# src-d/kmcuda

Hardware: NVIDIA H100
Metric: kmeans_assign_points_per_sec (higher is better)
Workload: dtype f16 tensor-core filter (f32 accumulate) + f32 exact re-check

## Files before the change

kmcuda_b200/csrc/assign_tc.cu:

```cuda
#include <cuda.h>
#include <cuda_fp16.h>

#include <cstdio>
#include <algorithm>
#include <cstring>
#include <map>
#include <mutex>
#include <tuple>
#include <vector>

#include <cub/cub.cuh>

#include "exact.cuh"
#include "kernels.h"
#include "sm90_ptx.cuh"

namespace kmb {

namespace tc {
constexpr int TM = 128;
constexpr int TN = 128;
constexpr int KB = 64;
constexpr int MAX_NKB = 8;
constexpr int WIDE_NKB = 4;
constexpr int B_STAGES = 4;
constexpr int A_KB_BYTES = TM * 128;
constexpr int B_KB_BYTES = TN * 128;
constexpr int B_STAGE_BYTES = B_KB_BYTES;
constexpr int AUG_A_BYTES = TM * 32;
constexpr int AUG_B_BYTES = TN * 32;
constexpr int LIST_LEN = 5;
#ifndef KMB_KO
#define KMB_KO 0
#endif
#ifndef KMB_PREP_FUSED
#define KMB_PREP_FUSED 1
#endif
constexpr int FIRST_EMIT_WARP = 0;
constexpr int FIRST_CONV_WARP = 4;
constexpr int FIRST_EPI_WARP = 8;
constexpr int WARP_B_PRODUCER = 16;
constexpr int N_CONV_WARPS = 4;
constexpr int N_EPI_WARPS = 8;
constexpr int N_EMIT_WARPS = 4;
constexpr int N_THREADS = 17 * 32;
constexpr int MAX_CAND = 32;
constexpr int KNN_CAP = 40;
constexpr int KNN_MAX_KK = 16;
constexpr float SENTINEL_GUARD = -65000.f;

enum { CNT_PAIRS = 0, CNT_ROWQ = 1, CNT_OVF = 2, CNT_ERR = 3, CNT_N = 4 };

struct Stats {
  float scale;
  float cmax;
  float dcmax;
  uint32_t csq_max_bits;
  uint32_t force_exact;
  float yabs;
  float mun;
  float knn_extra;
};

constexpr uint32_t LIST_ARRAY = 2 * LIST_LEN * 256 * 4;
struct SmemLayout {
  uint32_t a, b, aug_a, aug_b, list, norms, fin, mu, bars, total;
};

__host__ __device__ constexpr bool wide_nkb(int nkb) { return nkb > WIDE_NKB; }
__host__ __device__ constexpr int b_stages(int nkb) { return wide_nkb(nkb) ? 2 : B_STAGES; }
__host__ __device__ constexpr int aug_bufs(int nkb) { return nkb <= 2 ? 2 : 1; }
__host__ __device__ constexpr int a_slots(int nkb) { return nkb <= 2 ? 4 : nkb == 3 ? 5 : nkb == 4 ? 6 : MAX_NKB; }
__host__ __device__ constexpr int norm_depth(int nkb) { return a_slots(nkb) / nkb + 1; }

__host__ __device__ constexpr SmemLayout smem_layout(int nkb) {
  SmemLayout L{};
  uint32_t o = 0;
  L.a = o; o += a_slots(nkb) * A_KB_BYTES;
  L.b = o; o += b_stages(nkb) * B_STAGE_BYTES;
  L.aug_a = o; o += AUG_A_BYTES;
  L.aug_b = o; o += aug_bufs(nkb) * AUG_B_BYTES;
  L.list = o; o += 4 * LIST_ARRAY;
  L.fin = o; o += 2 * 5 * 256 * 4;
  L.norms = o; o += norm_depth(nkb) * 4 * TM * 4;
  L.mu = o; o += MAX_NKB * KB * 4;
  L.bars = o; o += 64 * 8;
  L.total = o;
  return L;
}
static_assert(4 * LIST_ARRAY + 2 * 5 * 256 * 4 >= 48 * 256 * 4, "k-NN scratch overlaps the norms");
__host__ __device__ constexpr bool layouts_fit() {
  for (int k = 1; k <= MAX_NKB; k++)
    if (smem_layout(k).total + 1024 > 232448 || a_slots(k) < k || a_slots(k) > MAX_NKB || norm_depth(k) * k <= a_slots(k))
      return false;
  return true;
}
static_assert(layouts_fit(), "227 KiB of shared memory per block on H100; a whole tile in the A ring; norms ring depth");

enum {
  BAR_B_FULL = 0,
  BAR_B_EMPTY = BAR_B_FULL + B_STAGES,
  BAR_AUG_FULL = BAR_B_EMPTY + B_STAGES,
  BAR_AUG_EMPTY = BAR_AUG_FULL + 2,
  BAR_A_FULL = BAR_AUG_EMPTY + 2,
  BAR_A_FREE = BAR_A_FULL + MAX_NKB,
  BAR_EMIT_FULL = BAR_A_FREE + MAX_NKB,
  BAR_EMIT_EMPTY = BAR_EMIT_FULL + 2,
  BAR_COUNT = BAR_EMIT_EMPTY + 2
};
static_assert(BAR_COUNT <= 63, "barrier array too small");

struct Params {
  uint32_t n;
  int D;
  uint32_t K;
  int nkb;
  int nt;
  uint32_t ntiles;
  const __half* aug_blob;
  const Stats* stats;
  uint32_t* result;
  uint32_t* pair_row;
  uint32_t* pair_cand;
  uint32_t max_pairs;
  uint32_t* rowq;
  uint32_t* ovf_rows;
  uint32_t* counters;
  int metric;
  const float* neg_mu_s;
  uint32_t* assign;
  uint32_t* prev;
  uint32_t* d_changed;
  const uint32_t* yy_qgroup;
  const uint32_t* yy_groups;
  const uint32_t* yy_assign;
  float* yy_bounds;
  uint32_t G;
  const float* X;
  const uint32_t* rows;
  const uint32_t* d_nrows;
  const uint32_t* d_ntiles;
  const uint32_t* tile_nrows;
  const uint32_t* blk_cluster;
// ... 360 lines not shown
      const float v = __ldcg(a.csq + c);
      if (v == v && v < 3.0e38f) best = max(best, __float_as_uint(fmaxf(v, 0.f)));
    }
    for (int o = 16; o > 0; o >>= 1) best = max(best, __shfl_xor_sync(0xffffffffu, best, o));
    if (lane == 0 && best) atomicMax(&a.stats->csq_max_bits, best);
    prep_grid_barrier(a.barrier, gridDim.x);
  }

  const bool have_mu = a.metric == 0 && a.centred;
  if (warp == 0) {
    float cmax = __fsqrt_ru(__uint_as_float(__ldcg(&a.stats->csq_max_bits)));
    float s = 1.f;
    if (cmax > 0.f && cmax < 3.0e38f) {
      int e;
      frexpf(cmax, &e);
      s = ldexpf(1.f, 6 - e);
    }
    if (lane == 0) s_scale = s;
    if (blockIdx.x == 0) {
      const int Dp = a.nkb * KB;
      float m2 = 0.f;
      for (int f = lane; f < Dp; f += 32) {
        const float m = (have_mu && f < D) ? s_mu[f] : 0.f;
        a.neg_mu_s[f] = -m * s;
        m2 = fmaf(m * s, m * s, m2);
      }
      for (int o = 16; o > 0; o >>= 1) m2 += __shfl_xor_sync(0xffffffffu, m2, o);
      if (lane == 0) {
        a.stats->scale = s;
        a.stats->cmax = cmax * s * 1.001f;
        a.stats->mun = __fsqrt_ru(m2) * 1.002f;
      }
    }
  }
  __syncthreads();
  const float s = s_scale;
  for (uint32_t row = gw; row < a.rows_pad; row += nw)
    prep_table_row(row, lane, s, a.metric, a.C, nsq, K, D, a.nkb, a.table, a.aug_blob, a.stats, a.gather,
                   have_mu ? s_mu : nullptr, a.by_source);
}

#define TC_WAIT(bar, parity, site) \
  ptx::mbar_wait(bars_u32 + 8u * static_cast<uint32_t>(bar), (parity), p.counters + CNT_ERR, site, bars_u32 + 8u * 63u)

__device__ __forceinline__ uint32_t commit_assignment(uint32_t* __restrict__ assign, uint32_t* __restrict__ prev,
                                                      uint64_t row, uint32_t winner) {
  const uint32_t a = assign[row];
  prev[row] = a;
  if (a == winner) return 0u;
  assign[row] = winner;
  return 1u;
}

__device__ __forceinline__ uint32_t compact_list(uint32_t* lst, uint32_t cnt, float thr) {
  constexpr uint32_t A = LIST_ARRAY / 4;
  uint32_t w = 0;
  for (uint32_t i = 0; i < cnt; i++) {
    const uint32_t cmb = lst[i * 256];
    if (__uint_as_float(cmb) >= thr) {
      if (w != i) {
        lst[w * 256] = cmb;
        lst[A + w * 256] = lst[A + i * 256];
        lst[2 * A + w * 256] = lst[2 * A + i * 256];
        lst[3 * A + w * 256] = lst[3 * A + i * 256];
      }
      w++;
    }
  }
  return w;
}

template <int MODE>
struct BlockIter {
  uint32_t cur, lo, hi, left;
  const uint2* rg;
  __device__ __forceinline__ BlockIter(const Params& p, uint32_t tile) {
    if (MODE == 2) {
      left = p.knn_nblk[tile];
      rg = p.knn_ranges + p.knn_roff[tile];
      if (left) { lo = cur = rg->x; hi = rg->y; } else { lo = cur = hi = 0; }
    } else {
      left = static_cast<uint32_t>(p.nt);
      lo = cur = 0;
      hi = left - 1;
      rg = nullptr;
    }
  }
  __device__ __forceinline__ bool valid() const { return left != 0; }
  __device__ __forceinline__ bool seg_first() const { return cur == lo; }
  __device__ __forceinline__ bool seg_last() const { return cur == hi; }
  __device__ __forceinline__ void next() {
    left--;
    if (MODE != 2) { cur++; return; }
    if (cur == hi && left) { rg++; lo = cur = rg->x; hi = rg->y; } else { cur++; }
  }
};

__device__ __noinline__ float knn_topk_insert(float* col, int kk, float v) {
  int j = kk - 1;
  while (j > 0 && col[(j - 1) * 256] < v) {
    col[j * 256] = col[(j - 1) * 256];
    j--;
  }
  col[j * 256] = v;
  return col[(kk - 1) * 256];
}
__device__ __noinline__ void knn_select_buckets(const float* mine, const float* partner, int kk, float goff,
                                                float* out) {
  unsigned long long taken = 0ull;
  for (int o = 0; o < kk; o++) {
    float best = -INFINITY;
    int bi = -1;
    for (int j = 0; j < 64; j++) {
      const float v = j < 32 ? mine[j * 256] : partner[(j - 32) * 256];
      if (!((taken >> j) & 1ull) && v > best) { best = v; bi = j; }
    }
    if (bi >= 0) taken |= 1ull << bi;
// ... 193 lines not shown
                nx2 = ptx::ffma2(b23, b23, nx2);
                const uint64_t d01 = ptx::fsub2(a01, b01), d23 = ptx::fsub2(a23, b23);
                nd2 = ptx::ffma2(d01, d01, nd2);
                nd2 = ptx::ffma2(d23, d23, nd2);
              } else {
                nx2 = ptx::ffma2(a01, a01, nx2);
                nx2 = ptx::ffma2(a23, a23, nx2);
              }
              if (MODE == 2) {
                const float q4 = fmaf(a0, a0, fmaf(a1, a1, fmaf(a2_, a2_, a3 * a3)));
                const float y = q4 - a2c, t = a2 + y;
                a2c = (t - a2) - y;
                a2 = t;
              }
              pk[half * 16 + c * 2] = *reinterpret_cast<uint32_t*>(&h0);
              pk[half * 16 + c * 2 + 1] = *reinterpret_cast<uint32_t*>(&h1);
            }
          }
          TC_WAIT(BAR_A_FREE + as, aph ^ 1, 7);
#if KMB_KO != 3
          uint8_t* a_row = smem + L.a + as * A_KB_BYTES + row * 128;
#pragma unroll
          for (int c = 0; c < 8; c++)
            *reinterpret_cast<uint4*>(a_row + ((c ^ (row & 7)) << 4)) =
                make_uint4(pk[4 * c], pk[4 * c + 1], pk[4 * c + 2], pk[4 * c + 3]);
#else
          (void)pk;
#endif
          if (kb == nkb - 1) {
            float* norms = reinterpret_cast<float*>(smem + L.norms) + (si % NDEPTH) * 4 * TM;
            float nxl, nxh, ndl, ndh;
            ptx::unpack2(nx2, nxl, nxh);
            ptx::unpack2(nd2, ndl, ndh);
            norms[row] = nxl + nxh;
            if (MEASURED_RESIDUAL) norms[TM + row] = ndl + ndh;
            if (MODE == 2) {
              norms[2 * TM + row] = a2;
              norms[3 * TM + row] = nraw * s * s;
            }
          }
          ptx::fence_proxy_async_smem();
          __syncwarp();
          if (lane == 0) ptx::mbar_arrive(&bars[BAR_A_FULL + as]);
          if (++as == ASLOTS) { as = 0; aph ^= 1; }
        }
      }
    }
  } else if (warp >= FIRST_EPI_WARP && warp < FIRST_EPI_WARP + N_EPI_WARPS) {
    const int e = warp - FIRST_EPI_WARP;
    const int g = e >> 2, wq = e & 3;
    const int h = (lane & 3) >> 1;
    const int row = g * 64 + wq * 16 + (lane >> 2) + 8 * (lane & 1);
    const int slot = h * TM + row;
    const uint64_t adesc0 = ptx::make_smem_desc(ptx::smem_u32(smem + L.a + g * (64 * 128)), 16, 1024, 1);
    const uint64_t bdesc0 = ptx::make_smem_desc(ptx::smem_u32(smem + L.b), 16, 1024, 1);
    const uint64_t aug_ad = ptx::make_smem_desc(ptx::smem_u32(smem + L.aug_a + g * 1024), TM * 16, 128, 0);
    const uint64_t aug_bd0 = ptx::make_smem_desc(ptx::smem_u32(smem + L.aug_b), TN * 16, 128, 0);
    uint32_t bs = 0, bph = 0;
    uint32_t a_ready_si = 0xFFFFFFFFu;
    uint32_t a0 = 0, aph0 = 0;
    const float cmax = p.stats->cmax, dcmax = p.stats->dcmax;
    const float mun = MODE == 2 ? 0.f : p.stats->mun;
    const float knn_extra = MODE == 2 ? p.stats->knn_extra : 0.f;
    const float cap = p.metric == 1 ? p.stats->scale * p.stats->scale : INFINITY;
    uint32_t ac = 0, ti = 0, si = 0;
    for (uint32_t tile = tile_begin; tile < tile_end; tile += gridDim.x) {
      if (MODE == 2 && p.knn_nblk[tile] == 0) continue;
      const int par = ti & 1;
      uint32_t* lst = reinterpret_cast<uint32_t*>(smem + L.list) + par * LIST_LEN * 256 + slot;
      float* fin = reinterpret_cast<float*>(smem + L.fin) + par * 5 * 256;
      if (MODE < 2) TC_WAIT(BAR_EMIT_EMPTY + par, ((ti >> 1) & 1) ^ 1, 11);
      float M = -INFINITY, M2 = -INFINITY, margin = 0.f;
      uint32_t cnt = 0, flags = 0;
      float* topk = reinterpret_cast<float*>(smem + L.list) + slot;
      uint32_t kslot = 0;
      bool klive = false;
      uint4* kent = nullptr;
      float goff = 0.f, mmax = 0.f;
      float xa2lo = 0.f;
      uint32_t gown = UINT32_MAX;
      uint32_t* yb = nullptr;
      bool ylive = false;
      if (MODE == 3) {
        const uint64_t grow = static_cast<uint64_t>(tile) * TM + row;
        ylive = grow < p.n;
        if (ylive) {
          const uint32_t a = p.yy_assign[grow];
          if (a < p.K) gown = p.yy_groups[a];
          yb = reinterpret_cast<uint32_t*>(p.yy_bounds + grow * (p.G + 1) + 1);
        }
      }
      uint32_t seg = 0;
      if (MODE == 2) {
        klive = static_cast<uint32_t>(row) < p.tile_nrows[tile];
        kslot = (tile * TM + row) * 2u + h;
        kent = p.knn_entries + static_cast<size_t>(kslot) * KNN_CAP;
        if (p.knn_first_pass || !klive) {
          for (int j = 0; j < p.kk; j++) topk[j * 256] = -INFINITY;
          if (p.knn_first_pass)
            for (int j = 0; j < 32; j++) topk[(16 + j) * 256] = -INFINITY;
        } else {
          for (int j = 0; j < p.kk; j++) topk[j * 256] = p.knn_topk[static_cast<size_t>(j) * p.knn_stride + kslot];
          cnt = p.knn_cnt[kslot];
          flags = p.knn_flags[kslot];
        }
        M = topk[(p.kk - 1) * 256];
      }
      for (BlockIter<MODE> it(p, tile); it.valid(); it.next(), ac++) {
        const int n = static_cast<int>(it.cur);
        const int buf = ac % AUGB;
        const uint32_t aph = (ac / AUGB) & 1;
        const bool need_a = a_ready_si != si;
        const bool free_a = it.seg_last();
        a_ready_si = si;
        __syncwarp();
        float acc[64];
        uint32_t sa_prev = 0;
#pragma unroll
        for (int kb = 0; kb < NKB; kb++) {
          const bool wrap = a0 + kb >= static_cast<uint32_t>(ASLOTS);
          const uint32_t sa = wrap ? a0 + kb - ASLOTS : a0 + kb;
          if (need_a) TC_WAIT(BAR_A_FULL + sa, wrap ? aph0 ^ 1 : aph0, 4);
          TC_WAIT(BAR_B_FULL + bs, bph, 5);
          __syncwarp();
#if KMB_KO != 2
          ptx::wgmma_fence_acc(acc);
          ptx::wgmma_fence();
          const uint64_t ad = adesc0 + ((sa * A_KB_BYTES) >> 4);
          const uint64_t bd = bdesc0 + ((bs * B_STAGE_BYTES) >> 4);
#pragma unroll
          for (int k = 0; k < 4; k++) ptx::wgmma_m64n128k16(acc, ad + 2 * k, bd + 2 * k, (kb | k) ? 1u : 0u);
          ptx::wgmma_commit();
          ptx::wgmma_fence_acc(acc);
#endif
          if (kb > 0) {
            ptx::wgmma_wait<1>();
            if (lane == 0) {
              ptx::mbar_arrive(&bars[BAR_B_EMPTY + (bs ? bs - 1 : BST - 1)]);
              if (free_a) ptx::mbar_arrive(&bars[BAR_A_FREE + sa_prev]);
            }
          }
          sa_prev = sa;
          if (++bs == BST) { bs = 0; bph ^= 1; }
        }
        TC_WAIT(BAR_AUG_FULL + buf, aph, 6);
        __syncwarp();
#if KMB_KO != 2
        ptx::wgmma_fence_acc(acc);
        ptx::wgmma_fence();
        ptx::wgmma_m64n128k16(acc, aug_ad, aug_bd0 + buf * (AUG_B_BYTES >> 4), 1u);
        ptx::wgmma_commit();
#endif
        ptx::wgmma_wait<0>();
#if KMB_KO != 2
        ptx::wgmma_fence_acc(acc);
#endif
        if (lane == 0) {
          ptx::mbar_arrive(&bars[BAR_B_EMPTY + (bs ? bs - 1 : BST - 1)]);
          ptx::mbar_arrive(&bars[BAR_AUG_EMPTY + buf]);
          if (free_a) ptx::mbar_arrive(&bars[BAR_A_FREE + sa_prev]);
        }
        if (free_a) {
          a0 += NKB;
          if (a0 >= static_cast<uint32_t>(ASLOTS)) { a0 -= ASLOTS; aph0 ^= 1; }
        }
        uint32_t r0[32], r1[32];
#if KMB_KO != 1
        regroup_quad(acc, lane, r0, r1);
#else
        for (int jj = 0; jj < 32; jj++) {
          r0[jj] = __float_as_uint(-64.f * static_cast<float>(n * 128 + h * 64 + jj + 1));
          r1[jj] = __float_as_uint(-64.f * static_cast<float>(n * 128 + h * 64 + 32 + jj + 1));
        }
#endif
        if (it.seg_first()) {
          const float* norms = reinterpret_cast<const float*>(smem + L.norms) + (si % NDEPTH) * 4 * TM;
          float nx, nd;
          if (MEASURED_RESIDUAL) {
            nx = __fsqrt_ru(norms[row]) * 1.0001f;
            nd = __fsqrt_ru(norms[TM + row]) * 1.0001f;
          } else {
            const float na = __fsqrt_ru(norms[row]) * 1.0001f;
            nd = na * 4.8834e-4f + __fsqrt_ru(static_cast<float>(p.nkb * KB)) * 2.99e-8f;
            nx = na + nd;
            if (!(na < 65000.f)) flags |= 1u;
          }
          const float xn = nx + nd;
          float E = nx * dcmax + nd * cmax + nd * dcmax;
          E += static_cast<float>(p.nkb * KB + 16) * 2.4e-7f * nx * cmax;
          const float xu = xn + mun, cu = cmax + mun;
          if (MODE == 0) {
            E += 6.0e-7f * (cu * cu + xu * cu);
          } else if (MODE == 2) {
            E += 2.0e-6f * (cu * cu + xu * cu) + 2.0e-6f * xu * xu;
          } else {
            E += 2.0e-6f * (xn + cmax) * (xn + cmax) + 2.4e-7f * (xn * cmax + cmax * cmax);
          }
          if (MODE == 3) {
            xa2lo = norms[row] * (1.f - 1.0e-4f);
            if (!(nx * cmax < 6.0e4f)) flags |= 1u;
          }
          if (MODE == 2) {
            goff = 0.5f * norms[2 * TM + row];
            E += 1.2e-7f * (__fsqrt_ru(norms[3 * TM + row]) * cmax + p.stats->yabs * xn) + 4.8e-7f * (goff + xn * cmax);
          }
          margin = 2.f * E * 1.001f + 1e-30f;
          if (MODE == 2) margin += knn_extra;
          if (!(margin < 1.0e30f)) flags |= 1u;
          if (MODE == 2) {
            mmax = fmaxf(mmax, margin);
            if (p.knn_first_pass && seg == 1) {
              float mg[KNN_MAX_KK];
              __syncwarp();
              knn_select_buckets(topk + 16 * 256, reinterpret_cast<float*>(smem + L.list) + ((1 - h) * TM + row) + 16 * 256,
                                 p.kk, goff, mg);
              __syncwarp();
              for (int j = 0; j < p.kk; j++) topk[j * 256] = mg[j];
              M = mg[p.kk - 1];
            }
          }
        }
#ifdef KMB_DEBUG_SCORES
        if (MODE == 0 && p.dbg_scores) {
          const uint64_t grow = static_cast<uint64_t>(tile) * TM + row;
          float* dst = p.dbg_scores + grow * (static_cast<uint64_t>(nt) * TN) + n * TN + h * 64;
          for (int jj = 0; jj < 32; jj++) dst[jj] = __uint_as_float(r0[jj]);
          for (int jj = 0; jj < 32; jj++) dst[32 + jj] = __uint_as_float(r1[jj]);
        }
#endif
        if (MODE == 3) {
          float qm[16];
#pragma unroll
          for (int i = 0; i < 8; i++) {
            qm[i] = fmaxf(ptx::fmax3(__uint_as_float(r0[4 * i]), __uint_as_float(r0[4 * i + 1]), __uint_as_float(r0[4 * i + 2])),
                          __uint_as_float(r0[4 * i + 3]));
            qm[8 + i] = fmaxf(ptx::fmax3(__uint_as_float(r1[4 * i]), __uint_as_float(r1[4 * i + 1]), __uint_as_float(r1[4 * i + 2])),
                              __uint_as_float(r1[4 * i + 3]));
          }
          uint32_t gq[16];
          {
            const uint4* src = reinterpret_cast<const uint4*>(p.yy_qgroup) + (static_cast<size_t>(n) * 2 + h) * 4;
#pragma unroll
            for (int i = 0; i < 4; i++) {
              const uint4 v = __ldg(src + i);
              gq[4 * i] = v.x; gq[4 * i + 1] = v.y; gq[4 * i + 2] = v.z; gq[4 * i + 3] = v.w;
            }
          }
          const float Eb = 0.5f * margin;
          const float sc = p.stats->scale;
          const float inv_s = 1.f / sc, inv_s2 = inv_s * inv_s;
          const bool emit_ok = ylive && !(flags & 1u);
          float run = qm[0];
#pragma unroll
          for (int i = 1; i <= 16; i++) {
            if (i == 16 || gq[i] != gq[i - 1]) {
              const uint32_t g = gq[i - 1];
              if (emit_ok && g < p.G && g != gown) {
                float v;
                if (p.metric == 1) {
                  const float dot = fminf(1.f, fmaxf(-1.f, (run + Eb) * inv_s2));
                  v = fmaxf(0.f, acosf(dot) - 4.0e-6f);
                } else {
                  const float t = xa2lo - 2.f * (run + Eb);
                  v = t > 0.f ? __fsqrt_rd(t) * inv_s * (1.f - 4.0e-6f) : 0.f;
                }
                atomicMin(yb + g, __float_as_uint(v));
              }
              if (i < 16) run = qm[i];
            } else {
              run = fmaxf(run, qm[i]);
            }
          }
          if (it.seg_last()) si++;
          continue;
        }
        float t0[8], t1[8];
        float cm0, cm1;
#if KMB_KO == 7
        if (MODE == 0) {
          uint32_t x0 = 0, x1 = 0;
#pragma unroll
          for (int jj = 0; jj < 32; jj += 8) { x0 ^= r0[jj]; x1 ^= r1[jj]; }
          M = fmaxf(M, __uint_as_float(x0 & x1 & 0x3fffffffu));
          if (it.seg_last()) si++;
          continue;
        }
#endif
        if (MODE == 2) {
#pragma unroll
          for (int i = 0; i < 8; i++) {
            t0[i] = fmaxf(fmaxf(__uint_as_float(r0[4 * i]), __uint_as_float(r0[4 * i + 1])),
                          fmaxf(__uint_as_float(r0[4 * i + 2]), __uint_as_float(r0[4 * i + 3])));
            t1[i] = fmaxf(fmaxf(__uint_as_float(r1[4 * i]), __uint_as_float(r1[4 * i + 1])),
                          fmaxf(__uint_as_float(r1[4 * i + 2]), __uint_as_float(r1[4 * i + 3])));
          }
          cm0 = fmaxf(fmaxf(fmaxf(t0[0], t0[1]), fmaxf(t0[2], t0[3])), fmaxf(fmaxf(t0[4], t0[5]), fmaxf(t0[6], t0[7])));
          cm1 = fmaxf(fmaxf(fmaxf(t1[0], t1[1]), fmaxf(t1[2], t1[3])), fmaxf(fmaxf(t1[4], t1[5]), fmaxf(t1[6], t1[7])));
        } else {
          float u0[10], u1[10];
#pragma unroll
          for (int i = 0; i < 10; i++) {
            u0[i] = ptx::fmax3(__uint_as_float(r0[3 * i]), __uint_as_float(r0[3 * i + 1]), __uint_as_float(r0[3 * i + 2]));
            u1[i] = ptx::fmax3(__uint_as_float(r1[3 * i]), __uint_as_float(r1[3 * i + 1]), __uint_as_float(r1[3 * i + 2]));
          }
          const float w00 = ptx::fmax3(u0[0], u0[1], u0[2]), w01 = ptx::fmax3(u0[3], u0[4], u0[5]);
          const float w02 = ptx::fmax3(u0[6], u0[7], u0[8]), w03 = ptx::fmax3(u0[9], __uint_as_float(r0[30]), __uint_as_float(r0[31]));
          const float w10 = ptx::fmax3(u1[0], u1[1], u1[2]), w11 = ptx::fmax3(u1[3], u1[4], u1[5]);
          const float w12 = ptx::fmax3(u1[6], u1[7], u1[8]), w13 = ptx::fmax3(u1[9], __uint_as_float(r1[30]), __uint_as_float(r1[31]));
          cm0 = fmaxf(ptx::fmax3(w00, w01, w02), w03);
          cm1 = fmaxf(ptx::fmax3(w10, w11, w12), w13);
        }
        float thr;
        if (MODE == 0) {
          M = fmaxf(M, fmaxf(cm0, cm1));
          thr = fminf(M, cap) - margin;
        } else if (MODE == 1) {
          M2 = fmaxf(M2, fminf(M, cm0));
          M = fmaxf(M, cm0);
          M2 = fmaxf(M2, fminf(M, cm1));
          M = fmaxf(M, cm1);
          thr = fminf(M2, cap) - margin;
        } else {
          if (p.knn_first_pass && seg == 0) {
            float* bk = topk + (16 + 16 * (n & 1)) * 256;
#pragma unroll
            for (int i = 0; i < 8; i++) {
              bk[i * 256] = fmaxf(bk[i * 256], t0[i]);
              bk[(8 + i) * 256] = fmaxf(bk[(8 + i) * 256], t1[i]);
            }
          } else if (!p.knn_first_pass) {
            const float lim = M + goff;
            if (cm0 > lim) {
#pragma unroll
              for (int i = 0; i < 8; i++)
                if (t0[i] - goff > M) M = knn_topk_insert(topk, p.kk, t0[i] - goff);
            }
            if (cm1 > lim) {
#pragma unroll
              for (int i = 0; i < 8; i++)
                if (t1[i] - goff > M) M = knn_topk_insert(topk, p.kk, t1[i] - goff);
            }
          }
          thr = (M - margin) + goff;
        }
        uint32_t nc0, nc1;
        {
          const uint64_t nthr2 = ptx::pack2(-thr, -thr);
          uint32_t c00 = 0, c01 = 0, c10 = 0, c11 = 0;
#pragma unroll
          for (int jj = 0; jj < 32; jj += 2) {
            float x0, y0, x1, y1;
            ptx::unpack2(ptx::fadd2(ptx::pack2(__uint_as_float(r0[jj]), __uint_as_float(r0[jj + 1])), nthr2), x0, y0);
            ptx::unpack2(ptx::fadd2(ptx::pack2(__uint_as_float(r1[jj]), __uint_as_float(r1[jj + 1])), nthr2), x1, y1);
            if (jj < 16) {
              c00 = __funnelshift_l(__float_as_uint(x0), c00, 1);
              c00 = __funnelshift_l(__float_as_uint(y0), c00, 1);
              c10 = __funnelshift_l(__float_as_uint(x1), c10, 1);
              c10 = __funnelshift_l(__float_as_uint(y1), c10, 1);
            } else {
              c01 = __funnelshift_l(__float_as_uint(x0), c01, 1);
              c01 = __funnelshift_l(__float_as_uint(y0), c01, 1);
              c11 = __funnelshift_l(__float_as_uint(x1), c11, 1);
              c11 = __funnelshift_l(__float_as_uint(y1), c11, 1);
            }
          }
          nc0 = (c00 << 16) | c01;
          nc1 = (c10 << 16) | c11;
        }
        const uint32_t mask0 = __brev(~nc0), mask1 = __brev(~nc1);
        if (MODE == 2) {
          if (klive && !(p.knn_first_pass && seg == 0)) {
            if (mask0)
              cnt = knn_append(kent, cnt, M, cm0 - goff, mask0, static_cast<uint32_t>(n) * 4 + h * 2, margin, &flags);
            if (mask1)
              cnt = knn_append(kent, cnt, M, cm1 - goff, mask1, static_cast<uint32_t>(n) * 4 + h * 2 + 1, margin, &flags);
          }
          if (it.seg_last()) { si++; seg++; }
          continue;
        }
        if (it.seg_last()) si++;
        if (mask0 | mask1) {
          constexpr uint32_t A = LIST_ARRAY / 4;
          if (cnt >= LIST_LEN - 1) cnt = compact_list(lst, cnt, thr);
          if (cnt < LIST_LEN) {
            lst[cnt * 256] = __float_as_uint(fmaxf(cm0, cm1));
            lst[A + cnt * 256] = mask0;
            lst[2 * A + cnt * 256] = mask1;
            lst[3 * A + cnt * 256] = static_cast<uint32_t>(n);
            cnt++;
          } else {
            flags |= 2u;
          }
        }
      }
      if (MODE == 2) {
        if (klive) {
          for (int j = 0; j < p.kk; j++) p.knn_topk[static_cast<size_t>(j) * p.knn_stride + kslot] = topk[j * 256];
          p.knn_cnt[kslot] = cnt;
          p.knn_flags[kslot] = flags;
          const float sc = p.stats->scale;
          const float d2 = fmaxf(0.f, -2.f * (M - mmax));
          p.knn_dub[kslot] = (M > -INFINITY && !flags) ? __fsqrt_ru(d2) / sc * 1.0001f : INFINITY;
        }
        ti++;
        continue;
      }
      if (MODE == 3) {
        if (ylive && (flags & 1u) && h == 0)
          p.ovf_rows[atomicAdd(&p.counters[CNT_OVF], 1u)] = static_cast<uint32_t>(tile * TM + row);
        ti++;
        continue;
      }
      fin[slot] = M;
      reinterpret_cast<uint32_t*>(fin)[256 + slot] = cnt;
      reinterpret_cast<uint32_t*>(fin)[512 + slot] = flags;
      fin[768 + slot] = margin;
      if (MODE == 1) fin[1024 + slot] = M2;
      __syncwarp();
      if (lane == 0) ptx::mbar_arrive(&bars[BAR_EMIT_FULL + par]);
      ti++;
    }
  } else if (warp >= FIRST_EMIT_WARP && warp < FIRST_EMIT_WARP + N_EMIT_WARPS && MODE < 2) {
    const int row = (warp - FIRST_EMIT_WARP) * 32 + lane;
    const float cap = p.metric == 1 ? p.stats->scale * p.stats->scale : INFINITY;
    const uint32_t force = p.stats->force_exact ? 16u : 0u;
    uint32_t ti = 0, nchanged = 0;
    for (uint32_t tile = tile_begin; tile < tile_end; tile += gridDim.x, ti++) {
      const int par = ti & 1;
      const uint32_t* lst = reinterpret_cast<const uint32_t*>(smem + L.list) + par * LIST_LEN * 256;
      const float* fin = reinterpret_cast<const float*>(smem + L.fin) + par * 5 * 256;
      const uint32_t* finu = reinterpret_cast<const uint32_t*>(fin);
      TC_WAIT(BAR_EMIT_FULL + par, (ti >> 1) & 1, 12);
      uint64_t grow = static_cast<uint64_t>(tile) * TM + row;
      uint32_t cand[MAX_CAND];
      uint32_t total = 0, fl = 0;
      const bool live = grow < n_eff;
      if (MODE == 1 && live) grow = p.rows[grow];
      if (live) {
        float Mf = fmaxf(fin[row], fin[TM + row]);
        if (MODE == 1)
          Mf = fmaxf(fminf(fin[row], fin[TM + row]), fmaxf(fin[1024 + row], fin[1024 + TM + row]));
        const float thr = fminf(Mf, cap) - fin[768 + row];
        fl = finu[512 + row] | finu[512 + TM + row] | force;
        if (p.metric == 1 && !(Mf >= fin[768 + row] - cap)) fl |= 8u;
        if (!(thr > SENTINEL_GUARD)) fl |= 8u;
        for (int hh = 0; hh < 2; hh++) {
          const int sl = hh * TM + row;
          const uint32_t c2 = finu[256 + sl];
          for (uint32_t i = 0; i < c2; i++) {
            constexpr uint32_t A = LIST_ARRAY / 4;
            if (!(__uint_as_float(lst[i * 256 + sl]) >= thr)) continue;
            const uint32_t base = lst[3 * A + i * 256 + sl] * TN + hh * 64;
#pragma unroll
            for (int c = 0; c < 2; c++) {
              uint32_t m = lst[(1 + c) * A + i * 256 + sl];
              while (m) {
                const int b = __ffs(m) - 1;
                m &= m - 1;
                const uint32_t col = base + c * 32 + b;
                if (col < p.K) {
                  if (total < MAX_CAND) cand[total] = col;
                  total++;
                }
              }
            }
          }
        }
      }
      __syncwarp();
      if (lane == 0) ptx::mbar_arrive(&bars[BAR_EMIT_EMPTY + par]);
      const bool overflow = live && (fl || total > MAX_CAND || (MODE == 1 && total == 0));
      const bool multi = live && !overflow && total >= (MODE == 1 ? 1u : 2u);
      uint32_t want = multi ? total : 0, pre = want;
#pragma unroll
      for (int o = 1; o < 32; o <<= 1) {
        uint32_t v = __shfl_up_sync(0xffffffffu, pre, o);
        if (lane >= o) pre += v;
      }
      const uint32_t warp_total = __shfl_sync(0xffffffffu, pre, 31);
      const unsigned mmask = __ballot_sync(0xffffffffu, multi);
      uint32_t base = 0, rqbase = 0;
      if (lane == 0 && warp_total) {
        base = atomicAdd(&p.counters[CNT_PAIRS], warp_total);
        rqbase = atomicAdd(&p.counters[CNT_ROWQ], static_cast<uint32_t>(__popc(mmask)));
      }
      base = __shfl_sync(0xffffffffu, base, 0) + (pre - want);
      rqbase = __shfl_sync(0xffffffffu, rqbase, 0) + __popc(mmask & ((1u << lane) - 1));
      if (live) {
        if (overflow) {
          p.ovf_rows[atomicAdd(&p.counters[CNT_OVF], 1u)] = static_cast<uint32_t>(grow);
        } else if (MODE == 0 && total == 1) {
          if (p.assign) nchanged += commit_assignment(p.assign, p.prev, grow, cand[0]);
          else p.result[grow] = cand[0];
        } else if (MODE == 0 && total == 0) {
          if (!p.assign) p.result[grow] = kUntouched;
        } else if (base + total <= p.max_pairs) {
          for (uint32_t i = 0; i < total; i++) {
            p.pair_row[base + i] = static_cast<uint32_t>(grow);
            p.pair_cand[base + i] = cand[i];
          }
          p.rowq[3 * rqbase] = static_cast<uint32_t>(grow);
          p.rowq[3 * rqbase + 1] = base;
          p.rowq[3 * rqbase + 2] = total;
        } else {
          p.rowq[3 * rqbase] = static_cast<uint32_t>(grow);
          p.rowq[3 * rqbase + 1] = 0;
          p.rowq[3 * rqbase + 2] = 0;
          p.ovf_rows[atomicAdd(&p.counters[CNT_OVF], 1u)] = static_cast<uint32_t>(grow);
        }
      }
    }
    if (MODE == 0 && p.assign) {
      nchanged = __reduce_add_sync(0xffffffffu, nchanged);
      if (lane == 0 && nchanged) atomicAdd(p.d_changed, nchanged);
    }
  }
// ... 1246 lines not shown
```

Before: 473.4 million.

## Filter scores in native MMA fragment layout, skipping the quad regroup

For the assign modes (MODE<2), the epilogue no longer regroups tensor-core accumulators through a quad shuffle. It computes column maxima, thresholds and candidate bitmasks directly on the native wgmma fragment layout, with per-row max reduced over the quad by shuffles. The candidate list and finalisation state are re-laid out per lane, each entry holding two row halves and a 16-bit tile id. The emit warps decode column indices from the interleaved fragment order by scanning four lane slots per row. This aims to remove the shuffle-heavy regroup and its register pressure, at the cost of more complex list bookkeeping and a larger shared-memory list area.

```diff
diff --git a/kmcuda_b200/csrc/assign_tc.cu b/kmcuda_b200/csrc/assign_tc.cu
--- a/kmcuda_b200/csrc/assign_tc.cu
+++ b/kmcuda_b200/csrc/assign_tc.cu
@@ -30,6 +30,7 @@
 constexpr int AUG_A_BYTES = TM * 32;
 constexpr int AUG_B_BYTES = TN * 32;
 constexpr int LIST_LEN = 5;
+constexpr int LIST_ARRAYS = 4;
 #ifndef KMB_KO
 #define KMB_KO 0
 #endif
@@ -63,6 +64,8 @@
 };
 
 constexpr uint32_t LIST_ARRAY = 2 * LIST_LEN * 256 * 4;
+constexpr uint32_t LIST_NT_BYTES = 2 * LIST_LEN * 256 * 2;
+enum { FIN_M = 0, FIN_MARGIN = TM, FIN_M2 = 2 * TM, FIN_STATE = 3 * TM, FIN_WORDS = 3 * TM + 256 };
 struct SmemLayout {
   uint32_t a, b, aug_a, aug_b, list, norms, fin, mu, bars, total;
 };
@@ -80,15 +83,15 @@
   L.b = o; o += b_stages(nkb) * B_STAGE_BYTES;
   L.aug_a = o; o += AUG_A_BYTES;
   L.aug_b = o; o += aug_bufs(nkb) * AUG_B_BYTES;
-  L.list = o; o += 4 * LIST_ARRAY;
-  L.fin = o; o += 2 * 5 * 256 * 4;
+  L.list = o; o += LIST_ARRAYS * LIST_ARRAY + LIST_NT_BYTES;
+  L.fin = o; o += 2 * FIN_WORDS * 4;
   L.norms = o; o += norm_depth(nkb) * 4 * TM * 4;
   L.mu = o; o += MAX_NKB * KB * 4;
   L.bars = o; o += 64 * 8;
   L.total = o;
   return L;
 }
-static_assert(4 * LIST_ARRAY + 2 * 5 * 256 * 4 >= 48 * 256 * 4, "k-NN scratch overlaps the norms");
+static_assert(LIST_ARRAYS * LIST_ARRAY + LIST_NT_BYTES + 2 * FIN_WORDS * 4 >= 48 * 256 * 4, "k-NN scratch overlaps the norms");
 __host__ __device__ constexpr bool layouts_fit() {
   for (int k = 1; k <= MAX_NKB; k++)
     if (smem_layout(k).total + 1024 > 232448 || a_slots(k) < k || a_slots(k) > MAX_NKB || norm_depth(k) * k <= a_slots(k))
@@ -555,17 +558,15 @@
   return 1u;
 }
 
-__device__ __forceinline__ uint32_t compact_list(uint32_t* lst, uint32_t cnt, float thr) {
+__device__ __forceinline__ uint32_t compact_list(uint32_t* lst, uint16_t* lnt, uint32_t cnt, float thr0, float thr1) {
   constexpr uint32_t A = LIST_ARRAY / 4;
   uint32_t w = 0;
+#pragma unroll 1
   for (uint32_t i = 0; i < cnt; i++) {
-    const uint32_t cmb = lst[i * 256];
-    if (__uint_as_float(cmb) >= thr) {
+    if (__uint_as_float(lst[i * 256]) >= thr0 || __uint_as_float(lst[A + i * 256]) >= thr1) {
       if (w != i) {
-        lst[w * 256] = cmb;
-        lst[A + w * 256] = lst[A + i * 256];
-        lst[2 * A + w * 256] = lst[2 * A + i * 256];
-        lst[3 * A + w * 256] = lst[3 * A + i * 256];
+        for (int k = 0; k < LIST_ARRAYS; k++) lst[k * A + w * 256] = lst[k * A + i * 256];
+        lnt[w * 256] = lnt[i * 256];
       }
       w++;
     }
@@ -865,6 +866,8 @@
     const int h = (lane & 3) >> 1;
     const int row = g * 64 + wq * 16 + (lane >> 2) + 8 * (lane & 1);
     const int slot = h * TM + row;
+    const int qrow = g * 64 + wq * 16 + (lane >> 2);
+    const int lid = e * 32 + lane;
     const uint64_t adesc0 = ptx::make_smem_desc(ptx::smem_u32(smem + L.a + g * (64 * 128)), 16, 1024, 1);
     const uint64_t bdesc0 = ptx::make_smem_desc(ptx::smem_u32(smem + L.b), 16, 1024, 1);
     const uint64_t aug_ad = ptx::make_smem_desc(ptx::smem_u32(smem + L.aug_a + g * 1024), TM * 16, 128, 0);
@@ -872,18 +875,19 @@
     uint32_t bs = 0, bph = 0;
     uint32_t a_ready_si = 0xFFFFFFFFu;
     uint32_t a0 = 0, aph0 = 0;
-    const float cmax = p.stats->cmax, dcmax = p.stats->dcmax;
-    const float mun = MODE == 2 ? 0.f : p.stats->mun;
-    const float knn_extra = MODE == 2 ? p.stats->knn_extra : 0.f;
     const float cap = p.metric == 1 ? p.stats->scale * p.stats->scale : INFINITY;
     uint32_t ac = 0, ti = 0, si = 0;
     for (uint32_t tile = tile_begin; tile < tile_end; tile += gridDim.x) {
       if (MODE == 2 && p.knn_nblk[tile] == 0) continue;
       const int par = ti & 1;
-      uint32_t* lst = reinterpret_cast<uint32_t*>(smem + L.list) + par * LIST_LEN * 256 + slot;
-      float* fin = reinterpret_cast<float*>(smem + L.fin) + par * 5 * 256;
+      uint32_t* lst = reinterpret_cast<uint32_t*>(smem + L.list) + par * LIST_LEN * 256 + lid;
+      uint16_t* lnt = reinterpret_cast<uint16_t*>(smem + L.list + LIST_ARRAYS * LIST_ARRAY) + par * LIST_LEN * 256 + lid;
+      float* fin = reinterpret_cast<float*>(smem + L.fin) + par * FIN_WORDS;
       if (MODE < 2) TC_WAIT(BAR_EMIT_EMPTY + par, ((ti >> 1) & 1) ^ 1, 11);
-      float M = -INFINITY, M2 = -INFINITY, margin = 0.f;
+      float M = -INFINITY, margin = 0.f;
+      float Mr[2] = {-INFINITY, -INFINITY}, M2r[2] = {-INFINITY, -INFINITY};
+      uint32_t* const fst = reinterpret_cast<uint32_t*>(fin) + FIN_STATE + lid;
+      if (MODE < 2) *fst = 0u;
       uint32_t cnt = 0, flags = 0;
       float* topk = reinterpret_cast<float*>(smem + L.list) + slot;
       uint32_t kslot = 0;
@@ -977,49 +981,66 @@
           a0 += NKB;
           if (a0 >= static_cast<uint32_t>(ASLOTS)) { a0 -= ASLOTS; aph0 ^= 1; }
         }
-        uint32_t r0[32], r1[32];
-#if KMB_KO != 1
-        regroup_quad(acc, lane, r0, r1);
-#else
-        for (int jj = 0; jj < 32; jj++) {
-          r0[jj] = __float_as_uint(-64.f * static_cast<float>(n * 128 + h * 64 + jj + 1));
-          r1[jj] = __float_as_uint(-64.f * static_cast<float>(n * 128 + h * 64 + 32 + jj + 1));
-        }
+#if KMB_KO == 1
+        if (MODE < 2)
+#pragma unroll
+          for (int j = 0; j < 16; j++)
+#pragma unroll
+            for (int q = 0; q < 4; q++)
+              acc[j * 4 + q] = -64.f * static_cast<float>(n * TN + 8 * j + 2 * (lane & 3) + (q & 1) + 1);
 #endif
         if (it.seg_first()) {
           const float* norms = reinterpret_cast<const float*>(smem + L.norms) + (si % NDEPTH) * 4 * TM;
-          float nx, nd;
-          if (MEASURED_RESIDUAL) {
-            nx = __fsqrt_ru(norms[row]) * 1.0001f;
-            nd = __fsqrt_ru(norms[TM + row]) * 1.0001f;
+          const float cmax = p.stats->cmax, dcmax = p.stats->dcmax;
+          const float mun = MODE == 2 ? 0.f : p.stats->mun;
+          const float knn_extra = MODE == 2 ? p.stats->knn_extra : 0.f;
+          auto row_margin = [&](int r, uint32_t& fl) {
+            float nx, nd;
+            if (MEASURED_RESIDUAL) {
+              nx = __fsqrt_ru(norms[r]) * 1.0001f;
+              nd = __fsqrt_ru(norms[TM + r]) * 1.0001f;
+            } else {
+              const float na = __fsqrt_ru(norms[r]) * 1.0001f;
+              nd = na * 4.8834e-4f + __fsqrt_ru(static_cast<float>(p.nkb * KB)) * 2.99e-8f;
+              nx = na + nd;
+              if (!(na < 65000.f)) fl |= 1u;
+            }
+            const float xn = nx + nd;
+            float E = nx * dcmax + nd * cmax + nd * dcmax;
+            E += static_cast<float>(p.nkb * KB + 16) * 2.4e-7f * nx * cmax;
+            const float xu = xn + mun, cu = cmax + mun;
+            if (MODE == 0) {
+              E += 6.0e-7f * (cu * cu + xu * cu);
+            } else if (MODE == 2) {
+              E += 2.0e-6f * (cu * cu + xu * cu) + 2.0e-6f * xu * xu;
+            } else {
+              E += 2.0e-6f * (xn + cmax) * (xn + cmax) + 2.4e-7f * (xn * cmax + cmax * cmax);
+            }
+            if (MODE == 3) {
+              xa2lo = norms[r] * (1.f - 1.0e-4f);
+              if (!(nx * cmax < 6.0e4f)) fl |= 1u;
+            }
+            if (MODE == 2) {
+              goff = 0.5f * norms[2 * TM + r];
+              E += 1.2e-7f * (__fsqrt_ru(norms[3 * TM + r]) * cmax + p.stats->yabs * xn) + 4.8e-7f * (goff + xn * cmax);
+            }
+            float mg = 2.f * E * 1.001f + 1e-30f;
+            if (MODE == 2) mg += knn_extra;
+            if (!(mg < 1.0e30f)) fl |= 1u;
+            return mg;
+          };
+          if (MODE < 2) {
+#pragma unroll
+            for (int hh = 0; hh < 2; hh++) {
+              uint32_t fl = 0;
+              const float mg = row_margin(qrow + 8 * hh, fl);
+              if ((lane & 3) == 0) fin[FIN_MARGIN + qrow + 8 * hh] = mg;
+              *fst |= fl << (8 + 8 * hh);
+            }
+            __syncwarp();
           } else {
-            const float na = __fsqrt_ru(norms[row]) * 1.0001f;
-            nd = na * 4.8834e-4f + __fsqrt_ru(static_cast<float>(p.nkb * KB)) * 2.99e-8f;
-            nx = na + nd;
-            if (!(na < 65000.f)) flags |= 1u;
+            margin = row_margin(row, flags);
           }
-          const float xn = nx + nd;
-          float E = nx * dcmax + nd * cmax + nd * dcmax;
-          E += static_cast<float>(p.nkb * KB + 16) * 2.4e-7f * nx * cmax;
-          const float xu = xn + mun, cu = cmax + mun;
-          if (MODE == 0) {
-            E += 6.0e-7f * (cu * cu + xu * cu);
-          } else if (MODE == 2) {
-            E += 2.0e-6f * (cu * cu + xu * cu) + 2.0e-6f * xu * xu;
-          } else {
-            E += 2.0e-6f * (xn + cmax) * (xn + cmax) + 2.4e-7f * (xn * cmax + cmax * cmax);
-          }
-          if (MODE == 3) {
-            xa2lo = norms[row] * (1.f - 1.0e-4f);
-            if (!(nx * cmax < 6.0e4f)) flags |= 1u;
-          }
-          if (MODE == 2) {
-            goff = 0.5f * norms[2 * TM + row];
-            E += 1.2e-7f * (__fsqrt_ru(norms[3 * TM + row]) * cmax + p.stats->yabs * xn) + 4.8e-7f * (goff + xn * cmax);
-          }
-          margin = 2.f * E * 1.001f + 1e-30f;
-          if (MODE == 2) margin += knn_extra;
-          if (!(margin < 1.0e30f)) flags |= 1u;
           if (MODE == 2) {
             mmax = fmaxf(mmax, margin);
             if (p.knn_first_pass && seg == 1) {
@@ -1033,12 +1054,94 @@
             }
           }
         }
+        if (MODE < 2) {
 #ifdef KMB_DEBUG_SCORES
-        if (MODE == 0 && p.dbg_scores) {
-          const uint64_t grow = static_cast<uint64_t>(tile) * TM + row;
-          float* dst = p.dbg_scores + grow * (static_cast<uint64_t>(nt) * TN) + n * TN + h * 64;
-          for (int jj = 0; jj < 32; jj++) dst[jj] = __uint_as_float(r0[jj]);
-          for (int jj = 0; jj < 32; jj++) dst[32 + jj] = __uint_as_float(r1[jj]);
+          if (MODE == 0 && p.dbg_scores)
+            for (int hh = 0; hh < 2; hh++) {
+              const uint64_t grow = static_cast<uint64_t>(tile) * TM + qrow + 8 * hh;
+              float* dst = p.dbg_scores + grow * (static_cast<uint64_t>(nt) * TN) + n * TN + 2 * (lane & 3);
+              for (int j = 0; j < 16; j++) {
+                dst[8 * j] = acc[j * 4 + hh * 2];
+                dst[8 * j + 1] = acc[j * 4 + hh * 2 + 1];
+              }
+            }
+#endif
+          if (it.seg_last()) si++;
+#if KMB_KO == 7
+          if (MODE == 0) {
+            uint32_t x0 = 0, x1 = 0;
+#pragma unroll
+            for (int j = 0; j < 16; j += 4) { x0 ^= __float_as_uint(acc[j * 4]); x1 ^= __float_as_uint(acc[j * 4 + 2]); }
+            Mr[0] = fmaxf(Mr[0], __uint_as_float(x0 & 0x3fffffffu));
+            Mr[1] = fmaxf(Mr[1], __uint_as_float(x1 & 0x3fffffffu));
+            continue;
+          }
+#endif
+          float cm[2], thr[2];
+          uint32_t mask[2];
+#pragma unroll
+          for (int hh = 0; hh < 2; hh++) {
+            auto v = [&](int b) { return acc[(b >> 1) * 4 + hh * 2 + (b & 1)]; };
+            float u[10];
+#pragma unroll
+            for (int i = 0; i < 10; i++) u[i] = ptx::fmax3(v(3 * i), v(3 * i + 1), v(3 * i + 2));
+            cm[hh] = fmaxf(ptx::fmax3(ptx::fmax3(u[0], u[1], u[2]), ptx::fmax3(u[3], u[4], u[5]), ptx::fmax3(u[6], u[7], u[8])),
+                           ptx::fmax3(u[9], v(30), v(31)));
+            if (MODE == 0) {
+              float qm = fmaxf(cm[hh], __shfl_xor_sync(0xffffffffu, cm[hh], 1));
+              qm = fmaxf(qm, __shfl_xor_sync(0xffffffffu, qm, 2));
+              Mr[hh] = fmaxf(Mr[hh], qm);
+              thr[hh] = fminf(Mr[hh], cap) - fin[FIN_MARGIN + qrow + 8 * hh];
+            } else {
+              const float o = __shfl_xor_sync(0xffffffffu, cm[hh], 1);
+              const float a1 = fmaxf(cm[hh], o), a2 = fminf(cm[hh], o);
+              const float b1 = __shfl_xor_sync(0xffffffffu, a1, 2), b2 = __shfl_xor_sync(0xffffffffu, a2, 2);
+              const float q1 = fmaxf(a1, b1), q2 = fmaxf(fminf(a1, b1), fmaxf(a2, b2));
+              M2r[hh] = ptx::fmax3(M2r[hh], q2, fminf(Mr[hh], q1));
+              Mr[hh] = fmaxf(Mr[hh], q1);
+              thr[hh] = fminf(M2r[hh], cap) - fin[FIN_MARGIN + qrow + 8 * hh];
+            }
+            const uint64_t nthr2 = ptx::pack2(-thr[hh], -thr[hh]);
+            uint32_t c0 = 0, c1 = 0;
+#pragma unroll
+            for (int j = 0; j < 16; j++) {
+              float x, y;
+              ptx::unpack2(ptx::fadd2(ptx::pack2(v(2 * j), v(2 * j + 1)), nthr2), x, y);
+              if (j < 8) {
+                c0 = __funnelshift_l(__float_as_uint(x), c0, 1);
+                c0 = __funnelshift_l(__float_as_uint(y), c0, 1);
+              } else {
+                c1 = __funnelshift_l(__float_as_uint(x), c1, 1);
+                c1 = __funnelshift_l(__float_as_uint(y), c1, 1);
+              }
+            }
+            mask[hh] = __brev(~((c0 << 16) | c1));
+          }
+          if (mask[0] | mask[1]) {
+            constexpr uint32_t A = LIST_ARRAY / 4;
+            uint32_t st = *fst, c = st & 0xffu;
+            if (c >= LIST_LEN - 1) c = compact_list(lst, lnt, c, thr[0], thr[1]);
+            if (c < LIST_LEN) {
+              lst[c * 256] = __float_as_uint(cm[0]);
+              lst[A + c * 256] = __float_as_uint(cm[1]);
+              lst[2 * A + c * 256] = mask[0];
+              lst[3 * A + c * 256] = mask[1];
+              lnt[c * 256] = static_cast<uint16_t>(n);
+              c++;
+            } else {
+              st |= (mask[0] ? 2u << 8 : 0u) | (mask[1] ? 2u << 16 : 0u);
+            }
+            *fst = (st & ~0xffu) | c;
+          }
+          continue;
+        }
+        uint32_t r0[32], r1[32];
+#if KMB_KO != 1
+        regroup_quad(acc, lane, r0, r1);
+#else
+        for (int jj = 0; jj < 32; jj++) {
+          r0[jj] = __float_as_uint(-64.f * static_cast<float>(n * 128 + h * 64 + jj + 1));
+          r1[jj] = __float_as_uint(-64.f * static_cast<float>(n * 128 + h * 64 + 32 + jj + 1));
         }
 #endif
         if (MODE == 3) {
@@ -1087,19 +1190,8 @@
           if (it.seg_last()) si++;
           continue;
         }
-        float t0[8], t1[8];
-        float cm0, cm1;
-#if KMB_KO == 7
-        if (MODE == 0) {
-          uint32_t x0 = 0, x1 = 0;
-#pragma unroll
-          for (int jj = 0; jj < 32; jj += 8) { x0 ^= r0[jj]; x1 ^= r1[jj]; }
-          M = fmaxf(M, __uint_as_float(x0 & x1 & 0x3fffffffu));
-          if (it.seg_last()) si++;
-          continue;
-        }
-#endif
         if (MODE == 2) {
+          float t0[8], t1[8];
 #pragma unroll
           for (int i = 0; i < 8; i++) {
             t0[i] = fmaxf(fmaxf(__uint_as_float(r0[4 * i]), __uint_as_float(r0[4 * i + 1])),
@@ -1107,33 +1199,8 @@
             t1[i] = fmaxf(fmaxf(__uint_as_float(r1[4 * i]), __uint_as_float(r1[4 * i + 1])),
                           fmaxf(__uint_as_float(r1[4 * i + 2]), __uint_as_float(r1[4 * i + 3])));
           }
-          cm0 = fmaxf(fmaxf(fmaxf(t0[0], t0[1]), fmaxf(t0[2], t0[3])), fmaxf(fmaxf(t0[4], t0[5]), fmaxf(t0[6], t0[7])));
-          cm1 = fmaxf(fmaxf(fmaxf(t1[0], t1[1]), fmaxf(t1[2], t1[3])), fmaxf(fmaxf(t1[4], t1[5]), fmaxf(t1[6], t1[7])));
-        } else {
-          float u0[10], u1[10];
-#pragma unroll
-          for (int i = 0; i < 10; i++) {
-            u0[i] = ptx::fmax3(__uint_as_float(r0[3 * i]), __uint_as_float(r0[3 * i + 1]), __uint_as_float(r0[3 * i + 2]));
-            u1[i] = ptx::fmax3(__uint_as_float(r1[3 * i]), __uint_as_float(r1[3 * i + 1]), __uint_as_float(r1[3 * i + 2]));
-          }
-          const float w00 = ptx::fmax3(u0[0], u0[1], u0[2]), w01 = ptx::fmax3(u0[3], u0[4], u0[5]);
-          const float w02 = ptx::fmax3(u0[6], u0[7], u0[8]), w03 = ptx::fmax3(u0[9], __uint_as_float(r0[30]), __uint_as_float(r0[31]));
-          const float w10 = ptx::fmax3(u1[0], u1[1], u1[2]), w11 = ptx::fmax3(u1[3], u1[4], u1[5]);
-          const float w12 = ptx::fmax3(u1[6], u1[7], u1[8]), w13 = ptx::fmax3(u1[9], __uint_as_float(r1[30]), __uint_as_float(r1[31]));
-          cm0 = fmaxf(ptx::fmax3(w00, w01, w02), w03);
-          cm1 = fmaxf(ptx::fmax3(w10, w11, w12), w13);
-        }
-        float thr;
-        if (MODE == 0) {
-          M = fmaxf(M, fmaxf(cm0, cm1));
-          thr = fminf(M, cap) - margin;
-        } else if (MODE == 1) {
-          M2 = fmaxf(M2, fminf(M, cm0));
-          M = fmaxf(M, cm0);
-          M2 = fmaxf(M2, fminf(M, cm1));
-          M = fmaxf(M, cm1);
-          thr = fminf(M2, cap) - margin;
-        } else {
+          const float cm0 = fmaxf(fmaxf(fmaxf(t0[0], t0[1]), fmaxf(t0[2], t0[3])), fmaxf(fmaxf(t0[4], t0[5]), fmaxf(t0[6], t0[7])));
+          const float cm1 = fmaxf(fmaxf(fmaxf(t1[0], t1[1]), fmaxf(t1[2], t1[3])), fmaxf(fmaxf(t1[4], t1[5]), fmaxf(t1[6], t1[7])));
           if (p.knn_first_pass && seg == 0) {
             float* bk = topk + (16 + 16 * (n & 1)) * 256;
 #pragma unroll
@@ -1154,34 +1221,32 @@
                 if (t1[i] - goff > M) M = knn_topk_insert(topk, p.kk, t1[i] - goff);
             }
           }
-          thr = (M - margin) + goff;
-        }
-        uint32_t nc0, nc1;
-        {
-          const uint64_t nthr2 = ptx::pack2(-thr, -thr);
-          uint32_t c00 = 0, c01 = 0, c10 = 0, c11 = 0;
-#pragma unroll
-          for (int jj = 0; jj < 32; jj += 2) {
-            float x0, y0, x1, y1;
-            ptx::unpack2(ptx::fadd2(ptx::pack2(__uint_as_float(r0[jj]), __uint_as_float(r0[jj + 1])), nthr2), x0, y0);
-            ptx::unpack2(ptx::fadd2(ptx::pack2(__uint_as_float(r1[jj]), __uint_as_float(r1[jj + 1])), nthr2), x1, y1);
-            if (jj < 16) {
-              c00 = __funnelshift_l(__float_as_uint(x0), c00, 1);
-              c00 = __funnelshift_l(__float_as_uint(y0), c00, 1);
-              c10 = __funnelshift_l(__float_as_uint(x1), c10, 1);
-              c10 = __funnelshift_l(__float_as_uint(y1), c10, 1);
-            } else {
-              c01 = __funnelshift_l(__float_as_uint(x0), c01, 1);
-              c01 = __funnelshift_l(__float_as_uint(y0), c01, 1);
-              c11 = __funnelshift_l(__float_as_uint(x1), c11, 1);
-              c11 = __funnelshift_l(__float_as_uint(y1), c11, 1);
+          const float thr = (M - margin) + goff;
+          uint32_t nc0, nc1;
+          {
+            const uint64_t nthr2 = ptx::pack2(-thr, -thr);
+            uint32_t c00 = 0, c01 = 0, c10 = 0, c11 = 0;
+#pragma unroll
+            for (int jj = 0; jj < 32; jj += 2) {
+              float x0, y0, x1, y1;
+              ptx::unpack2(ptx::fadd2(ptx::pack2(__uint_as_float(r0[jj]), __uint_as_float(r0[jj + 1])), nthr2), x0, y0);
+              ptx::unpack2(ptx::fadd2(ptx::pack2(__uint_as_float(r1[jj]), __uint_as_float(r1[jj + 1])), nthr2), x1, y1);
+              if (jj < 16) {
+                c00 = __funnelshift_l(__float_as_uint(x0), c00, 1);
+                c00 = __funnelshift_l(__float_as_uint(y0), c00, 1);
+                c10 = __funnelshift_l(__float_as_uint(x1), c10, 1);
+                c10 = __funnelshift_l(__float_as_uint(y1), c10, 1);
+              } else {
+                c01 = __funnelshift_l(__float_as_uint(x0), c01, 1);
+                c01 = __funnelshift_l(__float_as_uint(y0), c01, 1);
+                c11 = __funnelshift_l(__float_as_uint(x1), c11, 1);
+                c11 = __funnelshift_l(__float_as_uint(y1), c11, 1);
+              }
             }
+            nc0 = (c00 << 16) | c01;
+            nc1 = (c10 << 16) | c11;
           }
-          nc0 = (c00 << 16) | c01;
-          nc1 = (c10 << 16) | c11;
-        }
-        const uint32_t mask0 = __brev(~nc0), mask1 = __brev(~nc1);
-        if (MODE == 2) {
+          const uint32_t mask0 = __brev(~nc0), mask1 = __brev(~nc1);
           if (klive && !(p.knn_first_pass && seg == 0)) {
             if (mask0)
               cnt = knn_append(kent, cnt, M, cm0 - goff, mask0, static_cast<uint32_t>(n) * 4 + h * 2, margin, &flags);
@@ -1189,21 +1254,6 @@
               cnt = knn_append(kent, cnt, M, cm1 - goff, mask1, static_cast<uint32_t>(n) * 4 + h * 2 + 1, margin, &flags);
           }
           if (it.seg_last()) { si++; seg++; }
-          continue;
-        }
-        if (it.seg_last()) si++;
-        if (mask0 | mask1) {
-          constexpr uint32_t A = LIST_ARRAY / 4;
-          if (cnt >= LIST_LEN - 1) cnt = compact_list(lst, cnt, thr);
-          if (cnt < LIST_LEN) {
-            lst[cnt * 256] = __float_as_uint(fmaxf(cm0, cm1));
-            lst[A + cnt * 256] = mask0;
-            lst[2 * A + cnt * 256] = mask1;
-            lst[3 * A + cnt * 256] = static_cast<uint32_t>(n);
-            cnt++;
-          } else {
-            flags |= 2u;
-          }
         }
       }
       if (MODE == 2) {
@@ -1224,11 +1274,13 @@
         ti++;
         continue;
       }
-      fin[slot] = M;
-      reinterpret_cast<uint32_t*>(fin)[256 + slot] = cnt;
-      reinterpret_cast<uint32_t*>(fin)[512 + slot] = flags;
-      fin[768 + slot] = margin;
-      if (MODE == 1) fin[1024 + slot] = M2;
+      if ((lane & 3) == 0) {
+#pragma unroll
+        for (int hh = 0; hh < 2; hh++) {
+          fin[FIN_M + qrow + 8 * hh] = Mr[hh];
+          if (MODE == 1) fin[FIN_M2 + qrow + 8 * hh] = M2r[hh];
+        }
+      }
       __syncwarp();
       if (lane == 0) ptx::mbar_arrive(&bars[BAR_EMIT_FULL + par]);
       ti++;
@@ -1241,7 +1293,8 @@
     for (uint32_t tile = tile_begin; tile < tile_end; tile += gridDim.x, ti++) {
       const int par = ti & 1;
       const uint32_t* lst = reinterpret_cast<const uint32_t*>(smem + L.list) + par * LIST_LEN * 256;
-      const float* fin = reinterpret_cast<const float*>(smem + L.fin) + par * 5 * 256;
+      const uint16_t* lnt = reinterpret_cast<const uint16_t*>(smem + L.list + LIST_ARRAYS * LIST_ARRAY) + par * LIST_LEN * 256;
+      const float* fin = reinterpret_cast<const float*>(smem + L.fin) + par * FIN_WORDS;
       const uint32_t* finu = reinterpret_cast<const uint32_t*>(fin);
       TC_WAIT(BAR_EMIT_FULL + par, (ti >> 1) & 1, 12);
       uint64_t grow = static_cast<uint64_t>(tile) * TM + row;
@@ -1250,31 +1303,31 @@
       const bool live = grow < n_eff;
       if (MODE == 1 && live) grow = p.rows[grow];
       if (live) {
-        float Mf = fmaxf(fin[row], fin[TM + row]);
-        if (MODE == 1)
-          Mf = fmaxf(fminf(fin[row], fin[TM + row]), fmaxf(fin[1024 + row], fin[1024 + TM + row]));
-        const float thr = fminf(Mf, cap) - fin[768 + row];
-        fl = finu[512 + row] | finu[512 + TM + row] | force;
-        if (p.metric == 1 && !(Mf >= fin[768 + row] - cap)) fl |= 8u;
+        const int hh = (row >> 3) & 1;
+        const int lid0 = (row >> 4) * 32 + (row & 7) * 4;
+        const float Mf = MODE == 1 ? fin[FIN_M2 + row] : fin[FIN_M + row];
+        const float mg = fin[FIN_MARGIN + row];
+        const float thr = fminf(Mf, cap) - mg;
+        fl = force;
+        if (p.metric == 1 && !(Mf >= mg - cap)) fl |= 8u;
         if (!(thr > SENTINEL_GUARD)) fl |= 8u;
-        for (int hh = 0; hh < 2; hh++) {
-          const int sl = hh * TM + row;
-          const uint32_t c2 = finu[256 + sl];
+        for (int t = 0; t < 4; t++) {
+          const int sl = lid0 + t;
+          const uint32_t st = finu[FIN_STATE + sl];
+          fl |= (st >> (8 + 8 * hh)) & 0xffu;
+          const uint32_t c2 = st & 0xffu;
           for (uint32_t i = 0; i < c2; i++) {
             constexpr uint32_t A = LIST_ARRAY / 4;
-            if (!(__uint_as_float(lst[i * 256 + sl]) >= thr)) continue;
-            const uint32_t base = lst[3 * A + i * 256 + sl] * TN + hh * 64;
-#pragma unroll
-            for (int c = 0; c < 2; c++) {
-              uint32_t m = lst[(1 + c) * A + i * 256 + sl];
-              while (m) {
-                const int b = __ffs(m) - 1;
-                m &= m - 1;
-                const uint32_t col = base + c * 32 + b;
-                if (col < p.K) {
-                  if (total < MAX_CAND) cand[total] = col;
-                  total++;
-                }
+            if (!(__uint_as_float(lst[hh * A + i * 256 + sl]) >= thr)) continue;
+            const uint32_t base = static_cast<uint32_t>(lnt[i * 256 + sl]) * TN + 2 * t;
+            uint32_t m = lst[(2 + hh) * A + i * 256 + sl];
+            while (m) {
+              const int b = __ffs(m) - 1;
+              m &= m - 1;
+              const uint32_t col = base + 8 * (b >> 1) + (b & 1);
+              if (col < p.K) {
+                if (total < MAX_CAND) cand[total] = col;
+                total++;
               }
             }
           }
```

New measurement: 527.5 million, median of 6. 1.11x the previous value.
